# liyi14/mx-DeepIM

Measured on NVIDIA H100. Metric: 480x640 4-iter pose refinements/sec, higher is better.
Workload: dtype fp16

## Files before the change

### mx-deepim_b200/csrc/conv_igemm.cuh

```cuda
#pragma once
#include <cuda.h>
#include <cuda_fp16.h>
#include "common.cuh"
#include "wgmma.cuh"

namespace dim {

struct ConvKParams {
  CUtensorMap a_map[4];
  CUtensorMap a_lo_map[4];
  CUtensorMap b_map;
  CUtensorMap b_lo_map;
  CUtensorMap out_map[2];
  const __nv_bfloat16 *in_hi, *in_lo;
  int in_cols;
  int KH, KW, stride, cchunks;
  int BW, BH, n_col_tiles;
  int Hq, Ho, Wo, Bn;
  int out_Hp, out_Wp, out_py, out_px, Cout;
  int kblocks;
  float slope;
  const float *bias;
  __nv_bfloat16 *out_hi, *out_lo;
  int in_off_r, in_off_c;
// ... 139 lines not shown

constexpr int kConv1Slack = 2048;


__device__ __forceinline__ int frag_row(int t) { return ((t >> 5) << 4) + ((t & 31) >> 2); }

__device__ __forceinline__ uint32_t pack2_bf16_lo(float v0, float v1, uint32_t hi) {
  return pack2_bf16(v0 - __uint_as_float(hi << 16), v1 - __uint_as_float(hi & 0xFFFF0000u));
}

template <bool SPLIT3, bool F16>
__device__ __forceinline__ void epi_pack(float v0, float v1, float b0, float b1, float slope, uint32_t &hi, uint32_t &lo) {
  v0 += b0;
  v1 += b1;
  v0 = v0 > 0.f ? v0 : v0 * slope;
  v1 = v1 > 0.f ? v1 : v1 * slope;
  if (F16) {
    hi = pack2_f16(v0, v1);
  } else {
    hi = pack2_bf16(v0, v1);
    if (SPLIT3) lo = pack2_bf16_lo(v0, v1, hi);
  }
}

template <bool SPLIT3, bool F16>
__device__ __forceinline__ void store_pair(float v0, float v1, float2 b, float slope, __nv_bfloat16 *out_hi, __nv_bfloat16 *out_lo,
                                           long long off) {
  uint32_t h, l = 0;
  epi_pack<SPLIT3, F16>(v0, v1, b.x, b.y, slope, h, l);
  *reinterpret_cast<uint32_t *>(out_hi + off) = h;
  if (SPLIT3) *reinterpret_cast<uint32_t *>(out_lo + off) = l;
}

template <bool SPLIT3>
__device__ __forceinline__ void store_pair_generic(float v0, float v1, const ConvKParams &p, int n, bool valid, long long off,
                                                   long long add_off, long long mask_off) {
  if (!valid || n >= p.Cout) return;
  if (p.bias) {
    v0 += __ldg(p.bias + n);
    v1 += __ldg(p.bias + n + 1);
  }
  if (p.addend.p) {
    const __nv_bfloat162 a = *reinterpret_cast<const __nv_bfloat162 *>(p.addend.p + add_off);
    if (SPLIT3) {
      const __nv_bfloat162 al = *reinterpret_cast<const __nv_bfloat162 *>(p.addend.lo + add_off);
      v0 += __low2float(a) + __low2float(al);
      v1 += __high2float(a) + __high2float(al);
    } else {
      v0 += __low2float(a);
      v1 += __high2float(a);
    }
  }
  if (p.mask.p) {
    if (n < p.mask_climit) {
      const __nv_bfloat162 m = *reinterpret_cast<const __nv_bfloat162 *>(p.mask.p + mask_off);
      if (!(__low2float(m) > 0.f)) v0 *= p.slope;
      if (!(__high2float(m) > 0.f)) v1 *= p.slope;
    }
  } else {
    v0 = v0 > 0.f ? v0 : v0 * p.slope;
    v1 = v1 > 0.f ? v1 : v1 * p.slope;
  }
  if (SPLIT3) {
    const uint32_t h = pack2_bf16(v0, v1);
    *reinterpret_cast<uint32_t *>(p.out_hi + off) = h;
    *reinterpret_cast<uint32_t *>(p.out_lo + off) = pack2_bf16_lo(v0, v1, h);
  } else {
    *reinterpret_cast<__nv_bfloat162 *>(p.out_hi + off) = __floats2bfloat162_rn(v0, v1);
  }
}

template <int BLOCK_N, int STAGES, bool SPLIT3, int EPI>
struct ConvSmem2 {
  static constexpr int A_BYTES = 128 * 64 * 2;
  static constexpr int B_BYTES = BLOCK_N * 64 * 2;
  static constexpr int NPREC = SPLIT3 ? 2 : 1;
  static constexpr int STAGE_BYTES = (A_BYTES + B_BYTES) * NPREC;
  static constexpr int RING_BYTES = STAGES * STAGE_BYTES;
  static constexpr int LIMIT = 227 * 1024, FIXED = 1024  + 256 ;
  static constexpr bool TMA_EPI = EPI == 0 && !SPLIT3;
  static constexpr int STG_GROUPS =
      !TMA_EPI ? 0 : (RING_BYTES + 2 * BLOCK_N * 128 + FIXED <= LIMIT ? BLOCK_N / 64 : BLOCK_N / 128);
  static constexpr int STG_ROUNDS = TMA_EPI ? BLOCK_N / 64 / STG_GROUPS : 0;
  static constexpr int STG_BYTES = STG_GROUPS * 8192;
  static constexpr int TOTAL = RING_BYTES + 2 * STG_BYTES + FIXED;
  static_assert(TOTAL <= LIMIT, "conv_igemm shared memory");
};

template <int BLOCK_N, int STAGES, bool SPLIT3, bool F16, int EPI = 0>
__global__ void __launch_bounds__(384, 1) conv_igemm_persistent_kernel(const __grid_constant__ ConvKParams p,
                                                                       const int total_tiles, const int n_tiles) {
  using S = ConvSmem2<BLOCK_N, STAGES, SPLIT3, EPI>;
  constexpr uint32_t SBO = 1024u;

  extern __shared__ uint8_t smem_raw[];
  uint8_t *smem = reinterpret_cast<uint8_t *>((reinterpret_cast<uintptr_t>(smem_raw) + 1023) & ~(uintptr_t)1023);
  uint8_t *stg = smem + S::RING_BYTES;
  uint64_t *full_bar = reinterpret_cast<uint64_t *>(stg + 2 * S::STG_BYTES);
  uint64_t *empty_bar = full_bar + STAGES;

  const int wgi = threadIdx.x >> 7, warp = threadIdx.x >> 5;

  if (threadIdx.x == 0) {
    for (int s = 0; s < STAGES; ++s) {
      ptx::mbar_init(&full_bar[s], 1);
      ptx::mbar_init(&empty_bar[s], 2);
    }
    ptx::fence_barrier_init();
    ptx::prefetch_tmap(&p.b_map);
    ptx::prefetch_tmap(&p.a_map[0]);
    if (S::TMA_EPI) ptx::prefetch_tmap(&p.out_map[0]);
  }
  __syncthreads();

  if (wgi == 0) {
    ptx::regs_producer();
    if (warp == 0) {
      const uint32_t tx = (uint32_t)(p.BW * p.BH * 64 * 2 + BLOCK_N * 64 * 2) * S::NPREC;
      int s = 0;
      uint32_t ph = 0;
      for (int tile = blockIdx.x; tile < total_tiles; tile += gridDim.x) {
        const int nt = tile % n_tiles, mt = tile / n_tiles;
        const int col_tile = mt % p.n_col_tiles, row_tile = mt / p.n_col_tiles;
        const int g0 = row_tile * p.BH, ow0 = col_tile * p.BW, n0 = nt * BLOCK_N;
        for (int kb = 0; kb < p.kblocks; ++kb) {
          ptx::mbar_wait(&empty_bar[s], ph ^ 1u);
// ... 3 lines not shown
          if (p.stride == 2) {
            view = ((kh & 1) << 1) | (kw & 1);
            dr = kh >> 1;
            dc = kw >> 1;
          }
          uint8_t *st = smem + s * S::STAGE_BYTES;
          if (EPI) { dr += p.in_off_r; dc += p.in_off_c; }
          if (ptx::elect_one()) {
            ptx::mbar_expect_tx_raw(&full_bar[s], tx);
            for (int pr = 0; pr < S::NPREC; ++pr) {
              uint8_t *sa = st + pr * (S::A_BYTES + S::B_BYTES);
              const CUtensorMap *am = pr ? &p.a_lo_map[view] : &p.a_map[view];
              ptx::tma_load_3d_raw(sa, am, &full_bar[s], cc * 64, ow0 + dc, g0 + dr);
              if (EPI == 0) ptx::tma_load_3d_raw(sa + S::A_BYTES / 2, am, &full_bar[s], cc * 64, ow0 + dc, g0 + dr + (p.BH >> 1));
              ptx::tma_load_2d_raw(sa + S::A_BYTES, pr ? &p.b_lo_map : &p.b_map, &full_bar[s], kb * 64, n0);
            }
          }
          __syncwarp();
          if (++s == STAGES) { s = 0; ph ^= 1u; }
        }
      }
    }
  } else {
    ptx::regs_consumer();
    const int t = threadIdx.x & 127;
    const int half = wgi - 1;
    const int q2 = (t & 3) * 2;
    const bool arriver = t == 0;
    const uint32_t base = ptx::smem_u32(smem);
    uint8_t *my_stg = stg + half * S::STG_BYTES;
    const int lane = t & 31;
    const uint32_t st_addr = ptx::smem_u32(my_stg) + (uint32_t)((16 * (t >> 5) + 8 * ((lane >> 3) & 1) + (lane & 7)) * 128);
    const uint32_t st_sw = (uint32_t)(((lane >> 4) & 1) ^ (lane & 7));
    float acc[BLOCK_N / 2];
    int s = 0;
    uint32_t ph = 0;
    for (int tile = blockIdx.x; tile < total_tiles; tile += gridDim.x) {
      int prev = -1;
      for (int kb = 0; kb < p.kblocks; ++kb) {
        ptx::mbar_wait(&full_bar[s], ph);
        const uint32_t a_hi = base + s * S::STAGE_BYTES + half * 8192;
        const uint32_t b_hi = base + s * S::STAGE_BYTES + S::A_BYTES;
        const uint64_t da0 = ptx::gmma_desc(a_hi, 16, SBO, ptx::kSW128), db0 = ptx::gmma_desc(b_hi, 16, SBO, ptx::kSW128);
        const uint64_t dal0 = da0 + ((S::A_BYTES + S::B_BYTES) >> 4), dbl0 = db0 + ((S::A_BYTES + S::B_BYTES) >> 4);
        wg::fence_acc(acc);
        wg::fence();
#pragma unroll
        for (int k = 0; k < 4; ++k) {
          const uint64_t da = da0 + (uint64_t)(2 * k), db = db0 + (uint64_t)(2 * k);
          wg::mma<BLOCK_N, F16, 0, 0>(acc, da, db, (kb > 0 || k > 0) ? 1u : 0u);
          if (SPLIT3) {
            wg::mma<BLOCK_N, false, 0, 0>(acc, dal0 + (uint64_t)(2 * k), db, 1u);
            wg::mma<BLOCK_N, false, 0, 0>(acc, da, dbl0 + (uint64_t)(2 * k), 1u);
          }
        }
        wg::commit();
        wg::wait<1>();
        wg::fence_acc(acc);
        if (prev >= 0 && arriver) ptx::mbar_arrive(&empty_bar[prev]);
        prev = s;
        if (++s == STAGES) { s = 0; ph ^= 1u; }
      }
      wg::wait<0>();
      wg::fence_acc(acc);
      if (prev >= 0 && arriver) ptx::mbar_arrive(&empty_bar[prev]);

      const int nt = tile % n_tiles, mt = tile / n_tiles;
      const int col_tile = mt % p.n_col_tiles, row_tile = mt / p.n_col_tiles;
      const int n0 = nt * BLOCK_N;
      if constexpr (S::TMA_EPI) {
        const int gs = row_tile * p.BH + half * (p.BH >> 1), ow0 = col_tile * p.BW;
        const int n_img = gs / p.Hq, oh = gs - n_img * p.Hq;
        const bool store0 = n_img < p.Bn && oh < p.Ho, store1 = n_img + 1 < p.Bn && oh + (p.BH >> 1) > p.Hq;
#pragma unroll
        for (int rd = 0; rd < S::STG_ROUNDS; ++rd) {
          if (arriver) ptx::bulk_wait_read0();
          ptx::named_bar_sync(1 + half, 128);
#pragma unroll
          for (int i = 0; i < S::STG_GROUPS * 4; ++i) {
            const int j = rd * S::STG_GROUPS * 8 + 2 * i;
            const float *bj = p.bias + n0 + 8 * j + q2;
            const float b0 = __ldg(bj), b1 = __ldg(bj + 1), b2 = __ldg(bj + 8), b3 = __ldg(bj + 9);
            uint32_t h[4], unused;
            epi_pack<false, F16>(acc[4 * j + 0], acc[4 * j + 1], b0, b1, p.slope, h[0], unused);
            epi_pack<false, F16>(acc[4 * j + 2], acc[4 * j + 3], b0, b1, p.slope, h[1], unused);
            epi_pack<false, F16>(acc[4 * j + 4], acc[4 * j + 5], b2, b3, p.slope, h[2], unused);
            epi_pack<false, F16>(acc[4 * j + 6], acc[4 * j + 7], b2, b3, p.slope, h[3], unused);
            ptx::stmatrix_x4(st_addr + (uint32_t)((i >> 2) * 8192) + (((uint32_t)(2 * (i & 3)) ^ st_sw) << 4), h);
          }
          ptx::fence_proxy_async();
          ptx::named_bar_sync(1 + half, 128);
          if (arriver && store0) {
            for (int q = 0; q < S::STG_GROUPS; ++q)
              ptx::tma_store_4d(&p.out_map[0], my_stg + q * 8192, n0 + (rd * S::STG_GROUPS + q) * 64, ow0, oh, n_img);
            ptx::bulk_commit();
          }
        }
        if (store1) {
#pragma unroll
          for (int rr = 0; rr < 2; ++rr) {
            const int lr = frag_row(t) + rr * 8, bh = lr / p.BW;
            const int oh1 = oh + bh - p.Hq, ow = ow0 + lr - bh * p.BW;
            if (lr < p.BW * (p.BH >> 1) && oh1 >= 0 && oh1 < p.Ho) {
// ... 102 lines not shown
    if (warp == 0 && n_rows > 0) {
      if (ptx::elect_one()) {
        ptx::mbar_expect_tx_raw(res_bar, (uint32_t)S::RES_BYTES);
        for (int kb = 0; kb < 16; ++kb) {
          ptx::tma_load_2d_raw(res + kb * S::TAP_BYTES, &p.b_map, res_bar, kb * 32, 0);
          if (SPLIT3) ptx::tma_load_2d_raw(res + (16 + kb) * S::TAP_BYTES, &p.b_lo_map, res_bar, kb * 32, 0);
        }
      }
      __syncwarp();
      const size_t plane = (size_t)p.in_cols * 16;
      const uint8_t *src_hi = reinterpret_cast<const uint8_t *>(p.in_hi) + (size_t)ow0 * 16;
      const uint8_t *src_lo = reinterpret_cast<const uint8_t *>(p.in_lo) + (size_t)ow0 * 16;
      for (int s = 0; s < n_strips; ++s) {
        const int slot = s % STAGES;
        ptx::mbar_wait(&empty_bar[slot], (((uint32_t)(s / STAGES)) & 1u) ^ 1u);
        uint8_t *st = ring + slot * S::STAGE_BYTES;
        if (g_lo + s >= rows_total) {
          if (ptx::elect_one()) ptx::mbar_arrive(&full_bar[slot]);
        } else if (ptx::elect_one()) {
          ptx::mbar_expect_tx_raw(&full_bar[slot], (uint32_t)(4 * S::PLANE_BYTES * S::NPREC));
          const size_t row = (size_t)(g_lo + s) * 4 * plane;
#pragma unroll
          for (int c = 0; c < 4; ++c) {
            ptx::bulk_load_raw(st + c * S::PLANE_BYTES, src_hi + row + c * plane, S::PLANE_BYTES, &full_bar[slot]);
            if (SPLIT3)
              ptx::bulk_load_raw(st + S::STRIP_BYTES + c * S::PLANE_BYTES, src_lo + row + c * plane, S::PLANE_BYTES, &full_bar[slot]);
          }
        }
        __syncwarp();
      }
    }
  } else if (n_rows > 0) {
    ptx::regs_consumer();
    const int set = wgi - 1, t = threadIdx.x & 127, lane = t & 31;
    const bool leader = t == 0;
    const int co = frag_row(t);
    const float b0 = __ldg(p.bias + co), b1 = __ldg(p.bias + co + 8);
    const uint32_t ring_a = ptx::smem_u32(ring);
    const uint64_t dring = ptx::gmma_desc(ring_a, S::PLANE_BYTES, 128, ptx::kNoSwizzle);
    const uint64_t dring3 = ptx::gmma_desc(ring_a, 2u * S::PLANE_BYTES, 128, ptx::kNoSwizzle) + 3u;
    const uint64_t lo_step = (uint64_t)(S::STRIP_BYTES >> 4);
    const uint64_t slot_step = (uint64_t)(S::STAGE_BYTES >> 4);
    const uint64_t kstep = (uint64_t)(2 * S::PLANE_BYTES >> 4);
    const uint64_t dres = ptx::gmma_desc(ptx::smem_u32(res), 16, 512, ptx::kSW64);
    const uint64_t dres_lo = dres + (uint64_t)((16 * S::TAP_BYTES) >> 4);
    uint8_t *my_stg = stg + set * S::NPREC * S::STG_BYTES;
    const int st_px = ((lane >> 4) << 3) + (lane & 7), st_chunk = 2 * (t >> 5) + ((lane >> 3) & 1);
    const uint32_t st_addr = ptx::smem_u32(my_stg) + (uint32_t)(st_px * 128 + ((st_chunk ^ (lane & 7)) << 4));
    ptx::mbar_wait(res_bar, 0);
    if (set == 1 && leader) ptx::mbar_arrive(&empty_bar[0]);
    for (int row = set; row < n_rows; row += 2) {
      float acc[N / 2];
#pragma unroll
      for (int dh = 0; dh < 4; ++dh) {
        const int s = row + dh;
        ptx::mbar_wait(&full_bar[s % STAGES], ((uint32_t)(s / STAGES)) & 1u);
      }
      wg::fence_acc(acc);
      wg::fence();
#pragma unroll
      for (int dh = 0; dh < 4; ++dh) {
        const uint64_t so = (uint64_t)((row + dh) % STAGES) * slot_step;
#pragma unroll
        for (int k = 0; k < 2; ++k) {
#pragma unroll
          for (int dw = 0; dw < 4; ++dw) {
            if ((dh == 3 || dw == 3) && k == 1) continue;
            const uint64_t db = (dw == 3 ? dring3 : dring + (uint64_t)dw + (uint64_t)k * kstep) + so;
            const uint64_t wo = (uint64_t)((dh * 4 + dw) * (S::TAP_BYTES >> 4) + 2 * k);
            wg::mma<N, F16, 0, 0>(acc, dres + wo, db, (dh | dw | k) ? 1u : 0u);
            if (SPLIT3) {
              wg::mma<N, false, 0, 0>(acc, dres + wo, db + lo_step, 1u);
              wg::mma<N, false, 0, 0>(acc, dres_lo + wo, db, 1u);
            }
          }
        }
      }
      wg::commit();
      wg::wait<0>();
      wg::fence_acc(acc);
      if (leader) {
        ptx::mbar_arrive(&empty_bar[row % STAGES]);
        ptx::mbar_arrive(&empty_bar[(row + 1) % STAGES]);
      }
      const int g = g_lo + row;
      const int n_img = g / p.Hq, oh = g - n_img * p.Hq;
      if (n_img < p.Bn && oh < p.Ho) {
        if (leader) ptx::bulk_wait_read0();
        ptx::named_bar_sync(1 + set, 128);
#pragma unroll
        for (int i = 0; i < N / 16; ++i) {
          uint32_t h[4], l[4] = {0, 0, 0, 0};
          epi_pack<SPLIT3, F16>(acc[8 * i + 0], acc[8 * i + 1], b0, b0, p.slope, h[0], l[0]);
          epi_pack<SPLIT3, F16>(acc[8 * i + 2], acc[8 * i + 3], b1, b1, p.slope, h[1], l[1]);
          epi_pack<SPLIT3, F16>(acc[8 * i + 4], acc[8 * i + 5], b0, b0, p.slope, h[2], l[2]);
          epi_pack<SPLIT3, F16>(acc[8 * i + 6], acc[8 * i + 7], b1, b1, p.slope, h[3], l[3]);
          ptx::stmatrix_x4_trans(st_addr + (uint32_t)(i * 16 * 128), h);
          if (SPLIT3) ptx::stmatrix_x4_trans(st_addr + (uint32_t)(S::STG_BYTES + i * 16 * 128), l);
        }
        ptx::fence_proxy_async();
        ptx::named_bar_sync(1 + set, 128);
        if (leader) {
#pragma unroll
          for (int q = 0; q < N / kConv1StoreN; ++q) {
            ptx::tma_store_4d(&p.out_map[0], my_stg + q * kConv1StoreN * 128, 0, ow0 + q * kConv1StoreN, oh, n_img);
            if (SPLIT3)
              ptx::tma_store_4d(&p.out_map[1], my_stg + S::STG_BYTES + q * kConv1StoreN * 128, 0, ow0 + q * kConv1StoreN, oh, n_img);
          }
          ptx::bulk_commit();
        }
      }
    }
    if (leader) ptx::bulk_wait0();
  }
}

template <int STAGES, bool SPLIT3, bool F16, int NB>
__global__ void __launch_bounds__(384, 1) conv1_rgbd_kernel(const __grid_constant__ ConvKParams p, const int rows_total,
                                                            const int rows_per_chunk, const int chunks_per_col,
                                                            const int strip_bytes ) {
  constexpr int NPREC = SPLIT3 ? 2 : 1;
  constexpr int TAP_BYTES = NB * 128, RES_BYTES = 16 * TAP_BYTES * NPREC;
  extern __shared__ uint8_t smem_raw[];
  uint8_t *smem = reinterpret_cast<uint8_t *>((reinterpret_cast<uintptr_t>(smem_raw) + 1023) & ~(uintptr_t)1023);
  uint8_t *res = smem;
  uint8_t *ring = smem + RES_BYTES;
  const int stage_bytes = strip_bytes * NPREC;
  uint64_t *full_bar = reinterpret_cast<uint64_t *>(ring + STAGES * stage_bytes + kConv1Slack);
  uint64_t *empty_bar = full_bar + STAGES;
  uint64_t *res_bar = empty_bar + STAGES;

  const int wgi = threadIdx.x >> 7, warp = threadIdx.x >> 5;
// ... 127 lines not shown
```

### mx-deepim_b200/csrc/net.cu

```cuda
#include <cuda_fp16.h>
#include <string.h>

#include <memory>
#include <mutex>

#include "launch.cuh"
#include "net_state.cuh"

namespace dim {

static void build_geometry(NetState *ns, int H, int W) {
  int h = H, w = W;
  for (int i = 0; i < 10; ++i) {
    const LayerSpec &s = kLayers[i];
    LayerGeom &g = ns->g[i];
    g.Cin = s.Cin; g.Cout = s.Cout; g.k = s.k; g.stride = s.stride; g.pad = s.pad;
    g.Hin = h; g.Win = w;
    g.Ho = (h + 2 * s.pad - s.k) / s.stride + 1;
    g.Wo = (w + 2 * s.pad - s.k) / s.stride + 1;
    if (g.Ho < 1) g.Ho = 1;
    if (g.Wo < 1) g.Wo = 1;
    int Hp = h + 2 * s.pad, Wp = w + 2 * s.pad;
    if (s.stride == 2) { Hp += Hp & 1; Wp += Wp & 1; }
    g.py = g.px = s.pad;
// ... 2 lines not shown
      g.rows = Hp / 2; g.cols = Wp / 2; g.Cbuf = 64;
      g.KH = g.KW = 4; g.stride_eff = 1; g.Ceff = 64; g.Hq = g.rows;
      g.BLOCK_K = 64; g.BLOCK_N = 64;
    } else if (i == 0) {
      g.rows = Hp / 2; g.cols = Wp / 2; g.Cbuf = 32;
      g.KH = g.KW = 4; g.stride_eff = 1; g.Ceff = 32; g.Hq = g.rows;
      g.BLOCK_K = 32; g.BLOCK_N = 64;
    } else {
      g.rows = Hp; g.cols = Wp; g.Cbuf = s.Cin;
      g.KH = g.KW = s.k; g.stride_eff = s.stride; g.Ceff = s.Cin;
      g.Hq = (s.stride == 2) ? Hp / 2 : Hp;
      g.BLOCK_K = 64; g.BLOCK_N = s.Cout >= 256 ? 256 : 128;
    }
    int best_bw = 0, best_score = -1;
    for (int pass = 0; pass < 2 && best_bw == 0; ++pass)
      for (int d = 1; d <= g.Wo && d <= 128; ++d) {
        if (g.Wo % d) continue;
        if (pass == 0 && d < 8) continue;
        const int score = d * (128 / d) * 1000 + d;
        if (score > best_score) { best_score = score; best_bw = d; }
      }
    if (best_bw == 0) best_bw = 1;
    g.BW = best_bw; g.BH = 128 / best_bw;
    g.n_col_tiles = g.Wo > 0 ? g.Wo / g.BW : 0;
    if (i == 0) {
      const int nt = cdiv(g.Wo, 128);
      g.BW = cdiv(g.Wo, nt); g.BH = 1; g.n_col_tiles = nt;
    }
    g.kblocks = g.KH * g.KW * (g.Ceff / g.BLOCK_K);
    h = g.Ho; w = g.Wo;
  }
}

typedef CUresult (*EncodeTiledFn)(CUtensorMap *, CUtensorMapDataType, cuuint32_t, void *, const cuuint64_t *,
                                  const cuuint64_t *, const cuuint32_t *, const cuuint32_t *, CUtensorMapInterleave,
                                  CUtensorMapSwizzle, CUtensorMapL2promotion, CUtensorMapFloatOOBfill);
static EncodeTiledFn get_encode() {
  static EncodeTiledFn fn = nullptr;
  if (!fn) {
    void *p = nullptr;
    cudaDriverEntryPointQueryResult q;
    if (cudaGetDriverEntryPoint("cuTensorMapEncodeTiled", &p, cudaEnableDefault, &q) == cudaSuccess &&
        q == cudaDriverEntryPointSuccess)
      fn = reinterpret_cast<EncodeTiledFn>(p);
  }
  return fn;
}

int encode_map(CUtensorMap *m, void *base, int rank, const uint64_t *dims, const uint64_t *strides_bytes,
                      const uint32_t *box, int block_k ) {
  EncodeTiledFn fn = get_encode();
  DIM_REQUIRE(fn != nullptr, "cuTensorMapEncodeTiled entry point not available (driver too old?)");
  cuuint64_t gd[5]; cuuint64_t gs[5]; cuuint32_t bx[5]; cuuint32_t es[5];
  for (int i = 0; i < rank; ++i) { gd[i] = dims[i]; bx[i] = box[i]; es[i] = 1; }
  for (int i = 0; i < rank - 1; ++i) gs[i] = strides_bytes[i];
  CUresult r = fn(m, CU_TENSOR_MAP_DATA_TYPE_BFLOAT16, (cuuint32_t)rank, base, gd, gs, bx, es,
                  CU_TENSOR_MAP_INTERLEAVE_NONE,
                  block_k == 64 ? CU_TENSOR_MAP_SWIZZLE_128B
                                : (block_k == 32 ? CU_TENSOR_MAP_SWIZZLE_64B : CU_TENSOR_MAP_SWIZZLE_NONE),
                  CU_TENSOR_MAP_L2_PROMOTION_L2_256B, CU_TENSOR_MAP_FLOAT_OOB_FILL_NONE);
  if (r != CUDA_SUCCESS) {
    set_error("cuTensorMapEncodeTiled failed with CUresult %d (rank %d dims %llu %llu %llu box %u %u %u)", (int)r, rank,
              (unsigned long long)dims[0], (unsigned long long)dims[1], (unsigned long long)(rank > 2 ? dims[2] : 0),
              box[0], box[1], rank > 2 ? box[2] : 0);
    return 3;
  }
  return 0;
}

static int build_maps(NetState *ns, int B, bool f16, TensorMaps &tm) {
  for (int i = 0; i < 10; ++i) {
    const LayerGeom &g = ns->g[i];
    ConvKParams &kp = tm.kp[i];
    memset(&kp, 0, sizeof(kp));
    for (int lo = 0; lo < 2; ++lo) {
      __nv_bfloat16 *base = lo ? ns->act_lo[i] : ns->act_hi[i];
      CUtensorMap *maps = lo ? kp.a_lo_map : kp.a_map;
      const uint32_t box[3] = {(uint32_t)g.BLOCK_K, (uint32_t)g.BW, (uint32_t)(g.BH / 2)};
      if (i == 0 && ns->input_depth) {
        const uint64_t dims[4] = {8, (uint64_t)g.cols, 8, (uint64_t)B * g.rows};
        const uint64_t str[3] = {16, (uint64_t)g.cols * 16, (uint64_t)g.cols * 128};
        const uint32_t box4[4] = {8, (uint32_t)(g.BW + 3), 8, 1};
        if (int rc = encode_map(&maps[0], base, 4, dims, str, box4, 0)) return rc;
        maps[1] = maps[2] = maps[3] = maps[0];
      } else if (i == 0) {
      } else if (g.stride_eff == 1) {
        const uint64_t dims[3] = {(uint64_t)g.Cbuf, (uint64_t)g.cols, (uint64_t)B * g.rows};
        const uint64_t str[2] = {(uint64_t)g.Cbuf * 2, (uint64_t)g.cols * g.Cbuf * 2};
        if (int rc = encode_map(&maps[0], base, 3, dims, str, box, g.BLOCK_K)) return rc;
        maps[1] = maps[2] = maps[3] = maps[0];
      } else {
        for (int ph = 0; ph < 2; ++ph)
          for (int pw = 0; pw < 2; ++pw) {
            const uint64_t dims[3] = {(uint64_t)g.Cbuf, (uint64_t)g.cols / 2, (uint64_t)B * g.rows / 2};
            const uint64_t str[2] = {(uint64_t)2 * g.Cbuf * 2, (uint64_t)2 * g.cols * g.Cbuf * 2};
            __nv_bfloat16 *vb = base + ((size_t)ph * g.cols + pw) * g.Cbuf;
            if (int rc = encode_map(&maps[(ph << 1) | pw], vb, 3, dims, str, box, g.BLOCK_K)) return rc;
          }
      }
    }
    {
      const uint64_t Ktot = (uint64_t)g.KH * g.KW * g.Ceff;
      const uint64_t dims[2] = {Ktot, (uint64_t)g.Cout};
      const uint64_t str[1] = {Ktot * 2};
      const uint32_t box[2] = {(uint32_t)g.BLOCK_K, (uint32_t)(i == 0 && ns->input_depth ? 16 : g.BLOCK_N)};
      __nv_bfloat16 *wop = f16 ? ns->w_f16[i] : ns->w_hi[i];
      if (int rc = encode_map(&kp.b_map, wop, 2, dims, str, box, g.BLOCK_K)) return rc;
      if (int rc = encode_map(&kp.b_lo_map, ns->w_lo[i], 2, dims, str, box, g.BLOCK_K)) return rc;
    }
    kp.KH = g.KH; kp.KW = g.KW; kp.stride = g.stride_eff; kp.cchunks = g.Ceff / g.BLOCK_K;
    kp.BW = g.BW; kp.BH = g.BH; kp.n_col_tiles = g.n_col_tiles;
    kp.Hq = g.Hq; kp.Ho = g.Ho; kp.Wo = g.Wo; kp.Bn = B;
    if (i < 9) {
      const LayerGeom &nx = ns->g[i + 1];
      kp.out_Hp = nx.rows; kp.out_Wp = nx.cols; kp.out_py = nx.py; kp.out_px = nx.px;
    } else {
      kp.out_Hp = g.Ho; kp.out_Wp = g.Wo; kp.out_py = 0; kp.out_px = 0;
    }
    kp.Cout = g.Cout;
    kp.kblocks = g.kblocks;
    kp.slope = 0.1f;
    kp.bias = ns->bias[i];
    kp.out_hi = ns->act_hi[i + 1];
    kp.out_lo = ns->act_lo[i + 1];
    if (i == 0 && !ns->input_depth) {
      kp.in_hi = ns->act_hi[0];
      kp.in_lo = ns->act_lo[0];
      kp.in_cols = g.cols;
    }
    if (i > 0 || !ns->input_depth) {
      DIM_REQUIRE(i == 0 || (g.BH % 2 == 0 && g.BH / 2 <= g.Hq && g.BW * (g.BH / 2) <= 64),
                  "conv_igemm: a consumer warpgroup's box must be whole output rows within two images");
      const uint64_t cb = (uint64_t)g.Cout * 2;
      const uint64_t dims[4] = {(uint64_t)g.Cout, (uint64_t)g.Wo, (uint64_t)g.Ho, (uint64_t)B};
      const uint64_t str[3] = {cb, (uint64_t)kp.out_Wp * cb, (uint64_t)kp.out_Hp * kp.out_Wp * cb};
      const uint32_t box[4] = {64, (uint32_t)(i == 0 ? kConv1StoreN : g.BW), (uint32_t)(i == 0 ? 1 : g.BH / 2), 1};
      const size_t interior = ((size_t)kp.out_py * kp.out_Wp + kp.out_px) * g.Cout;
      for (int lo = 0; lo < (i == 0 ? 2 : 1); ++lo)
        if (int rc = encode_map(&kp.out_map[lo], (lo ? ns->act_lo[i + 1] : ns->act_hi[i + 1]) + interior, 4, dims, str, box, 64))
          return rc;
    }
  }
  return 0;
}

template <bool F16>
__device__ __forceinline__ void mma_bf16_16816(float *c, const uint32_t *a, uint32_t b0, uint32_t b1) {
  if (F16)
    asm volatile(
        "mma.sync.aligned.m16n8k16.row.col.f32.f16.f16.f32 {%0,%1,%2,%3}, {%4,%5,%6,%7}, {%8,%9}, {%0,%1,%2,%3};"
        : "+f"(c[0]), "+f"(c[1]), "+f"(c[2]), "+f"(c[3])
        : "r"(a[0]), "r"(a[1]), "r"(a[2]), "r"(a[3]), "r"(b0), "r"(b1));
  else
    asm volatile(
        "mma.sync.aligned.m16n8k16.row.col.f32.bf16.bf16.f32 {%0,%1,%2,%3}, {%4,%5,%6,%7}, {%8,%9}, {%0,%1,%2,%3};"
        : "+f"(c[0]), "+f"(c[1]), "+f"(c[2]), "+f"(c[3])
        : "r"(a[0]), "r"(a[1]), "r"(a[2]), "r"(a[3]), "r"(b0), "r"(b1));
}

template <bool S3, bool F16 = false>
__global__ void __launch_bounds__(256) fc6_mma_kernel(const __nv_bfloat16 *__restrict__ act_hi,
                                                      const __nv_bfloat16 *__restrict__ act_lo,
                                                      const __nv_bfloat16 *__restrict__ w_hi,
                                                      const __nv_bfloat16 *__restrict__ w_lo, int B, int max_batch,
                                                      float *__restrict__ partial) {
  constexpr int PITCH = FC6_KC * 2 + 64;
  __shared__ __align__(16) uint8_t a_hi_s[16 * PITCH];
  __shared__ __align__(16) uint8_t a_lo_s[S3 ? 16 * PITCH : 16];
  const int s = blockIdx.x, k0 = s * FC6_KC;
// ... 273 lines not shown
  n[11] = 256 * 256;
  for (int i = 0; i < 12; ++i) off[i + 1] = off[i] + n[i];
  float *stage_p = nullptr;
  DIM_CHECK(cudaMalloc(&stage_p, off[12] * sizeof(float)));
  std::unique_ptr<float, cudaError_t (*)(void *)> stage(stage_p, cudaFree);
  auto put = [](float *dst, const float *src, size_t count) {
    return cudaMemcpy(dst, src, count * sizeof(float), cudaMemcpyHostToDevice);
  };
  const float *w[12];
  for (int i = 0; i < 12; ++i) {
    w[i] = stage.get() + off[i];
    if (i != 10) DIM_CHECK(put(stage.get() + off[i], W[i], n[i]));
  }
  {
    std::vector<float> p((size_t)256 * FC6_K);
    for (int o = 0; o < 256; ++o)
      for (int c = 0; c < 1024; ++c)
        for (int hw = 0; hw < 80; ++hw) p[(size_t)o * FC6_K + (size_t)hw * 1024 + c] = W[10][(size_t)o * FC6_K + (size_t)c * 80 + hw];
    DIM_CHECK(put(stage.get() + off[10], p.data(), n[10]));
  }
  for (int i = 0; i < 10; ++i) DIM_CHECK(put(ns->bias[i], Bv[i], ns->g[i].Cout));
  DIM_CHECK(put(ns->fc6_b, Bv[10], 256));
  DIM_CHECK(put(ns->fc7_b, Bv[11], 256));
  DIM_CHECK(put(ns->rot_w, W[12], 4 * 256));
  DIM_CHECK(put(ns->rot_b, Bv[12], 4));
  DIM_CHECK(put(ns->trans_w, W[13], 3 * 256));
  DIM_CHECK(put(ns->trans_b, Bv[13], 3));
  if (int rc = net_pack_weights(ctx, w, 0, true, true)) return rc;
  DIM_CHECK(cudaStreamSynchronize(0));
  ns->loaded = true;
  return 0;
}

template <int BN, int ST, bool S3, bool F16>
static int launch_conv(const ConvKParams &kp, int total_tiles, int n_tiles, int cap, cudaStream_t st) {
  using S = ConvSmem2<BN, ST, S3, 0>;
  static bool attr_set = false;
  if (!attr_set) {
    DIM_CHECK(cudaFuncSetAttribute(conv_igemm_persistent_kernel<BN, ST, S3, F16>, cudaFuncAttributeMaxDynamicSharedMemorySize,
                                   S::TOTAL));
    attr_set = true;
  }
  const int grid = total_tiles < cap ? total_tiles : cap;
  conv_igemm_persistent_kernel<BN, ST, S3, F16><<<grid, 384, S::TOTAL, st>>>(kp, total_tiles, n_tiles);
  DIM_LAUNCH_CHECK();
  return 0;
}

template <int N, int ST, bool S3, bool F16>
static int launch_conv1(const ConvKParams &kp, int grid, int rows_total, int rpc, int chunks, cudaStream_t st) {
  using S = Conv1Smem<N, ST, S3>;
  static bool set = false;
  if (!set) {
    DIM_CHECK(cudaFuncSetAttribute(conv1_kernel<N, ST, S3, F16>, cudaFuncAttributeMaxDynamicSharedMemorySize, S::TOTAL));
    set = true;
  }
  conv1_kernel<N, ST, S3, F16><<<grid, 384, S::TOTAL, st>>>(kp, rows_total, rpc, chunks);
  DIM_LAUNCH_CHECK();
  return 0;
}

template <int ST, bool S3, bool F16, int NB>
static int launch_conv1_rgbd(const ConvKParams &kp, int grid, int rows_total, int rpc, int chunks, int strip_bytes,
                             cudaStream_t st) {
  const int smem_bytes = 16 * NB * 128 * (S3 ? 2 : 1) + ST * (S3 ? 2 : 1) * strip_bytes + kConv1Slack + 1024 + 256;
  DIM_REQUIRE(smem_bytes <= 227 * 1024, "conv1 (RGB-D): image too wide for the rolling-strip ring");
  static int set = 0;
  if (set < smem_bytes) {
    DIM_CHECK(cudaFuncSetAttribute(conv1_rgbd_kernel<ST, S3, F16, NB>, cudaFuncAttributeMaxDynamicSharedMemorySize,
                                   smem_bytes));
    set = smem_bytes;
  }
  conv1_rgbd_kernel<ST, S3, F16, NB><<<grid, 384, smem_bytes, st>>>(kp, rows_total, rpc, chunks, strip_bytes);
  DIM_LAUNCH_CHECK();
  return 0;
}

// ... 15 lines not shown
  }
  ns->act_hi[0] = enable ? ns->act0_rgbd_hi : ns->act0_rgb_hi;
  ns->act_lo[0] = enable ? ns->act0_rgbd_lo : ns->act0_rgb_lo;
  return 0;
}

bool net_input_depth(dim_ctx *ctx) { return ctx->net && ctx->net->input_depth; }

int net_set_input_mask(dim_ctx *ctx, bool enable) {
  NetState *ns = ctx->net;
  DIM_REQUIRE(ns != nullptr, "net not created");
  if (ns->input_mask == enable) return 0;
  DIM_REQUIRE(!ns->loaded, "dim_ctx_set_input_mask: call it before dim_net_load (this context's weights are loaded)");
  ns->input_mask = enable;
  return 0;
}

bool net_input_mask(dim_ctx *ctx) { return !ctx->net || ctx->net->input_mask; }

void net_input_geometry(dim_ctx *ctx, int *rows, int *cols, int *pad, __nv_bfloat16 **hi, __nv_bfloat16 **lo) {
  NetState *ns = ctx->net;
  *rows = ns->g[0].rows; *cols = ns->g[0].cols; *pad = ns->g[0].py;
  *hi = ns->act_hi[0]; *lo = ns->act_lo[0];
}

int net_forward(dim_ctx *ctx, int B, int precision, const float *zoom_factor, float *rot_out, float *trans_out,
                float *se3_out, cudaStream_t st, cudaEvent_t after_conv) {
  NetState *ns = ctx->net;
  DIM_REQUIRE(ns && ns->loaded, "dim_net_load has not been called");
  DIM_REQUIRE(B >= 1 && B <= ctx->max_batch, "batch exceeds max_batch");
  DIM_REQUIRE(precision == DIM_PREC_BF16 || precision == DIM_PREC_BF16X3 || precision == DIM_PREC_FP16,
              "unknown precision (DIM_PREC_BF16 / DIM_PREC_BF16X3 / DIM_PREC_FP16)");
  const bool s3 = precision == DIM_PREC_BF16X3, f16 = precision == DIM_PREC_FP16;
  const int key = B + (f16 ? kF16MapKey : 0);
  auto it = ns->maps.find(key);
  if (it == ns->maps.end()) {
    TensorMaps tm;
    if (int rc = build_maps(ns, B, f16, tm)) return rc;
    it = ns->maps.emplace(key, tm).first;
  }
  const TensorMaps &tm = it->second;
  if (ns->repack_done) DIM_CHECK(cudaStreamWaitEvent(st, ns->repack_done, 0));
  if (s3 && ns->lo_stale)
    if (int rc = train_refresh_lo(ctx, st)) return rc;
  if (f16 && ns->f16_stale)
    if (int rc = net_refresh_f16(ctx, st)) return rc;
  if (ns->layer_events) DIM_CHECK(cudaEventRecord(ns->layer_events[0], st));
  for (int i = 0; i < 10; ++i) {
    const LayerGeom &g = ns->g[i];
    const ConvKParams &kp = tm.kp[i];
    const int n_tiles = g.Cout / g.BLOCK_N;
    const int total_tiles = cdiv(B * g.Hq, g.BH) * g.n_col_tiles * n_tiles;
    const int sms = ctx->num_sms;
    int rc;
    if (i == 0 && ns->input_depth) {
      const int nsplit = s3 ? 4 : 1;
      const int rows_total = B * g.Hq;
      int chunks = sms / (g.n_col_tiles * nsplit);
      if (chunks > cdiv(rows_total, 16)) chunks = cdiv(rows_total, 16);
      if (chunks < 1) chunks = 1;
      const int rpc = cdiv(rows_total, chunks);
      chunks = cdiv(rows_total, rpc);
      const int strip_bytes = cdiv((g.BW + 3) * 128, 128) * 128;
      const int grid = g.n_col_tiles * chunks * nsplit;
      rc = s3 ? launch_conv1_rgbd<5, true, false, 16>(kp, grid, rows_total, rpc, chunks, strip_bytes, st)
              : (f16 ? launch_conv1_rgbd<6, false, true, 64>(kp, grid, rows_total, rpc, chunks, strip_bytes, st)
                     : launch_conv1_rgbd<6, false, false, 64>(kp, grid, rows_total, rpc, chunks, strip_bytes, st));
    } else if (i == 0) {
      DIM_REQUIRE(g.Wo == 320 && g.cols >= g.Wo + 3 && g.Hq == g.rows && g.Hq == g.Ho + 3,
                  "conv1_kernel is built for a 480x640 input (320 output columns)");
      const int n_col = g.Wo / (s3 ? 80 : 160);
      const int rows_total = B * g.Hq;
      int chunks = sms / n_col;
      if (chunks > cdiv(rows_total, 16)) chunks = cdiv(rows_total, 16);
      if (chunks < 1) chunks = 1;
      const int rpc = cdiv(rows_total, chunks);
      chunks = cdiv(rows_total, rpc);
      const int grid = n_col * chunks;
      rc = s3 ? launch_conv1<80, 5, true, false>(kp, grid, rows_total, rpc, chunks, st)
              : (f16 ? launch_conv1<160, 8, false, true>(kp, grid, rows_total, rpc, chunks, st)
                     : launch_conv1<160, 8, false, false>(kp, grid, rows_total, rpc, chunks, st));
    } else if (g.BLOCK_N == 128) {
      rc = s3 ? launch_conv<128, 3, true, false>(kp, total_tiles, n_tiles, sms, st)
              : (f16 ? launch_conv<128, 6, false, true>(kp, total_tiles, n_tiles, sms, st)
                     : launch_conv<128, 6, false, false>(kp, total_tiles, n_tiles, sms, st));
    } else {
      rc = s3 ? launch_conv<256, 2, true, false>(kp, total_tiles, n_tiles, sms, st)
              : (f16 ? launch_conv<256, 4, false, true>(kp, total_tiles, n_tiles, sms, st)
                     : launch_conv<256, 4, false, false>(kp, total_tiles, n_tiles, sms, st));
    }
    if (rc) return rc;
    if (ns->layer_events && i < 9) DIM_CHECK(cudaEventRecord(ns->layer_events[i + 1], st));
  }
  if (ns->layer_events) DIM_CHECK(cudaEventRecord(ns->layer_events[10], st));
  if (after_conv) DIM_CHECK(cudaEventRecord(after_conv, st));
  if (s3)
    fc6_mma_kernel<true><<<FC6_SPLITS, 256, 0, st>>>(ns->act_hi[10], ns->act_lo[10], ns->fc6_w_hi, ns->fc6_w_lo, B,
                                                     ctx->max_batch, ns->fc6_partial);
  else if (f16)
    fc6_mma_kernel<false, true><<<FC6_SPLITS, 256, 0, st>>>(ns->act_hi[10], nullptr, ns->fc6_w_f16, nullptr, B,
                                                            ctx->max_batch, ns->fc6_partial);
  else
    fc6_mma_kernel<false><<<FC6_SPLITS, 256, 0, st>>>(ns->act_hi[10], nullptr, ns->fc6_w_hi, nullptr, B,
                                                      ctx->max_batch, ns->fc6_partial);
  DIM_LAUNCH_CHECK();
  head_kernel<<<B, 1024, 0, st>>>(ns->fc6_partial, ctx->max_batch, ns->fc6_b, ns->fc7_wT, ns->fc7_b, ns->rot_w,
                                 ns->rot_b, ns->trans_w, ns->trans_b, zoom_factor, rot_out, trans_out, se3_out, ns->save_h6,
                                 ns->save_h7);
  DIM_LAUNCH_CHECK();
  return 0;
}

bool net_graph_safe(dim_ctx *ctx) {
  NetState *ns = ctx->net;
  return ns && ns->loaded && !ns->layer_events && !ns->train_aliased;
}

int net_layer_profile(dim_ctx *ctx, int enable, float *ms10) {
// ... 41 lines not shown
```

### mx-deepim_b200/csrc/net_state.cuh

```cuda
#pragma once
#include <map>

#include "conv_igemm.cuh"

namespace dim {

struct LayerSpec {
  const char *name;
  int Cout, Cin, k, stride, pad;
};
static const LayerSpec kLayers[10] = {
    {"flow_conv1", 64, 8, 7, 2, 3},  {"conv2", 128, 64, 5, 2, 2},   {"conv3", 256, 128, 5, 2, 2},
    {"conv3_1", 256, 256, 3, 1, 1},  {"conv4", 512, 256, 3, 2, 1},  {"conv4_1", 512, 512, 3, 1, 1},
    {"conv5", 512, 512, 3, 2, 1},    {"conv5_1", 512, 512, 3, 1, 1}, {"conv6", 1024, 512, 3, 2, 1},
    {"conv6_1", 1024, 1024, 3, 1, 1}};

struct LayerGeom {
  int Cin, Cout, k, stride, pad, Hin, Win, Ho, Wo;
  int rows, cols, Cbuf, py, px;
  int KH, KW, stride_eff, Ceff, Hq;
  int BLOCK_N, BLOCK_K, BW, BH, n_col_tiles, kblocks;
};

struct TensorMaps {
// ... 14 lines not shown
  LayerGeom g[10];
  __nv_bfloat16 *w_hi[10] = {}, *w_lo[10] = {};
  __nv_bfloat16 *w_f16[10] = {};
  float *bias[10] = {};
  __nv_bfloat16 *act_hi[11] = {}, *act_lo[11] = {};
  size_t act_elems_per_image[11] = {};
  __nv_bfloat16 *fc6_w_hi = nullptr, *fc6_w_lo = nullptr;
  __nv_bfloat16 *fc6_w_f16 = nullptr;
  bool train_aliased = false;
  bool f16_stale = false;
  float *fc6_b = nullptr, *fc7_wT = nullptr, *fc7_b = nullptr, *rot_w = nullptr, *rot_b = nullptr,
        *trans_w = nullptr, *trans_b = nullptr;
  float *fc6_partial = nullptr;
  cudaEvent_t *layer_events = nullptr;
  bool loaded = false, net_ok = false;
  bool input_depth = false;
  __nv_bfloat16 *act0_rgb_hi = nullptr, *act0_rgb_lo = nullptr, *act0_rgbd_hi = nullptr, *act0_rgbd_lo = nullptr;
  bool input_mask = true;
  float *save_h6 = nullptr, *save_h7 = nullptr;
  cudaEvent_t repack_done = nullptr;
  bool lo_stale = false;
  std::map<int, TensorMaps> maps;
  int max_batch = 0;
};

static constexpr int FC6_K = 1024 * 8 * 10;
static constexpr int FC6_KC = 256;
static constexpr int FC6_SPLITS = FC6_K / FC6_KC;


int encode_map(CUtensorMap *m, void *base, int rank, const uint64_t *dims, const uint64_t *strides_bytes,
               const uint32_t *box, int block_k );
static constexpr int kF16MapKey = 1 << 20;

}
```

Baseline: 3316.

## Transpose 128-channel conv GEMM so weights are M and 256 pixels are N

For 128-output-channel layers in fp16/bf16 forward mode, the implicit-GEMM kernel swaps operands: each consumer warpgroup takes 64 output channels as the MMA M dimension and a 256-pixel tile as N. The accumulator is written through stmatrix-transposed staging and TMA-stored one output row at a time. Doubling the pixel tile is meant to reuse each weight tile across more pixels and give larger wgmma N, at the cost of fewer pipeline stages (6 to 4), more accumulator registers, and per-row TMA stores issued by one thread. Tensor-map caching now keys on bf16x3 so the differing tile geometry stays separate.

```diff
diff --git a/mx-deepim_b200/csrc/conv_igemm.cuh b/mx-deepim_b200/csrc/conv_igemm.cuh
--- a/mx-deepim_b200/csrc/conv_igemm.cuh
+++ b/mx-deepim_b200/csrc/conv_igemm.cuh
@@ -195,6 +195,22 @@
   if (SPLIT3) *reinterpret_cast<uint32_t *>(out_lo + off) = l;
 }
 
+__device__ __forceinline__ uint32_t stage_trans_lane(int t) {
+  const int lane = t & 31;
+  const int px = ((lane >> 4) << 3) + (lane & 7), chunk = 2 * (t >> 5) + ((lane >> 3) & 1);
+  return (uint32_t)(px * 128 + ((chunk ^ (lane & 7)) << 4));
+}
+template <bool SPLIT3, bool F16>
+__device__ __forceinline__ void stage_trans16(const float *a, float b0, float b1, float slope, uint32_t addr, uint32_t lo_off) {
+  uint32_t h[4], l[4] = {0, 0, 0, 0};
+  epi_pack<SPLIT3, F16>(a[0], a[1], b0, b0, slope, h[0], l[0]);
+  epi_pack<SPLIT3, F16>(a[2], a[3], b1, b1, slope, h[1], l[1]);
+  epi_pack<SPLIT3, F16>(a[4], a[5], b0, b0, slope, h[2], l[2]);
+  epi_pack<SPLIT3, F16>(a[6], a[7], b1, b1, slope, h[3], l[3]);
+  ptx::stmatrix_x4_trans(addr, h);
+  if (SPLIT3) ptx::stmatrix_x4_trans(addr + lo_off, l);
+}
+
 template <bool SPLIT3>
 __device__ __forceinline__ void store_pair_generic(float v0, float v1, const ConvKParams &p, int n, bool valid, long long off,
                                                    long long add_off, long long mask_off) {
@@ -233,28 +249,32 @@
   }
 }
 
-template <int BLOCK_N, int STAGES, bool SPLIT3, int EPI>
+template <int BLOCK_N, int STAGES, bool SPLIT3, int EPI, bool TRANS = false>
 struct ConvSmem2 {
-  static constexpr int A_BYTES = 128 * 64 * 2;
+  static constexpr int TILE_PX = TRANS ? 256 : 128;
+  static constexpr int A_BYTES = TILE_PX * 64 * 2;
   static constexpr int B_BYTES = BLOCK_N * 64 * 2;
   static constexpr int NPREC = SPLIT3 ? 2 : 1;
   static constexpr int STAGE_BYTES = (A_BYTES + B_BYTES) * NPREC;
   static constexpr int RING_BYTES = STAGES * STAGE_BYTES;
   static constexpr int LIMIT = 227 * 1024, FIXED = 1024  + 256 ;
   static constexpr bool TMA_EPI = EPI == 0 && !SPLIT3;
+  static constexpr int OUT_BLOCKS = (TRANS ? TILE_PX : BLOCK_N) / 64;
   static constexpr int STG_GROUPS =
-      !TMA_EPI ? 0 : (RING_BYTES + 2 * BLOCK_N * 128 + FIXED <= LIMIT ? BLOCK_N / 64 : BLOCK_N / 128);
-  static constexpr int STG_ROUNDS = TMA_EPI ? BLOCK_N / 64 / STG_GROUPS : 0;
+      !TMA_EPI ? 0 : (RING_BYTES + 2 * OUT_BLOCKS * 8192 + FIXED <= LIMIT ? OUT_BLOCKS : OUT_BLOCKS / 2);
+  static constexpr int STG_ROUNDS = TMA_EPI ? OUT_BLOCKS / STG_GROUPS : 0;
   static constexpr int STG_BYTES = STG_GROUPS * 8192;
   static constexpr int TOTAL = RING_BYTES + 2 * STG_BYTES + FIXED;
   static_assert(TOTAL <= LIMIT, "conv_igemm shared memory");
+  static_assert(!TRANS || (BLOCK_N == 128 && TMA_EPI), "transposed tiles: 128 output channels, fp16 / bf16 forward");
 };
 
-template <int BLOCK_N, int STAGES, bool SPLIT3, bool F16, int EPI = 0>
+template <int BLOCK_N, int STAGES, bool SPLIT3, bool F16, int EPI = 0, bool TRANS = false>
 __global__ void __launch_bounds__(384, 1) conv_igemm_persistent_kernel(const __grid_constant__ ConvKParams p,
                                                                        const int total_tiles, const int n_tiles) {
-  using S = ConvSmem2<BLOCK_N, STAGES, SPLIT3, EPI>;
+  using S = ConvSmem2<BLOCK_N, STAGES, SPLIT3, EPI, TRANS>;
   constexpr uint32_t SBO = 1024u;
+  constexpr int MMA_N = TRANS ? S::TILE_PX : BLOCK_N;
 
   extern __shared__ uint8_t smem_raw[];
   uint8_t *smem = reinterpret_cast<uint8_t *>((reinterpret_cast<uintptr_t>(smem_raw) + 1023) & ~(uintptr_t)1023);
@@ -324,15 +344,17 @@
     const int lane = t & 31;
     const uint32_t st_addr = ptx::smem_u32(my_stg) + (uint32_t)((16 * (t >> 5) + 8 * ((lane >> 3) & 1) + (lane & 7)) * 128);
     const uint32_t st_sw = (uint32_t)(((lane >> 4) & 1) ^ (lane & 7));
-    float acc[BLOCK_N / 2];
+    const uint32_t st_trans = ptx::smem_u32(my_stg) + stage_trans_lane(t);
+    float acc[MMA_N / 2];
     int s = 0;
     uint32_t ph = 0;
     for (int tile = blockIdx.x; tile < total_tiles; tile += gridDim.x) {
       int prev = -1;
       for (int kb = 0; kb < p.kblocks; ++kb) {
         ptx::mbar_wait(&full_bar[s], ph);
-        const uint32_t a_hi = base + s * S::STAGE_BYTES + half * 8192;
-        const uint32_t b_hi = base + s * S::STAGE_BYTES + S::A_BYTES;
+        const uint32_t act = base + s * S::STAGE_BYTES, wts = act + S::A_BYTES;
+        const uint32_t a_hi = TRANS ? wts + half * 8192 : act + half * 8192;
+        const uint32_t b_hi = TRANS ? act : wts;
         const uint64_t da0 = ptx::gmma_desc(a_hi, 16, SBO, ptx::kSW128), db0 = ptx::gmma_desc(b_hi, 16, SBO, ptx::kSW128);
         const uint64_t dal0 = da0 + ((S::A_BYTES + S::B_BYTES) >> 4), dbl0 = db0 + ((S::A_BYTES + S::B_BYTES) >> 4);
         wg::fence_acc(acc);
@@ -340,10 +362,10 @@
 #pragma unroll
         for (int k = 0; k < 4; ++k) {
           const uint64_t da = da0 + (uint64_t)(2 * k), db = db0 + (uint64_t)(2 * k);
-          wg::mma<BLOCK_N, F16, 0, 0>(acc, da, db, (kb > 0 || k > 0) ? 1u : 0u);
+          wg::mma<MMA_N, F16, 0, 0>(acc, da, db, (kb > 0 || k > 0) ? 1u : 0u);
           if (SPLIT3) {
-            wg::mma<BLOCK_N, false, 0, 0>(acc, dal0 + (uint64_t)(2 * k), db, 1u);
-            wg::mma<BLOCK_N, false, 0, 0>(acc, da, dbl0 + (uint64_t)(2 * k), 1u);
+            wg::mma<MMA_N, false, 0, 0>(acc, dal0 + (uint64_t)(2 * k), db, 1u);
+            wg::mma<MMA_N, false, 0, 0>(acc, da, dbl0 + (uint64_t)(2 * k), 1u);
           }
         }
         wg::commit();
@@ -360,7 +382,29 @@
       const int nt = tile % n_tiles, mt = tile / n_tiles;
       const int col_tile = mt % p.n_col_tiles, row_tile = mt / p.n_col_tiles;
       const int n0 = nt * BLOCK_N;
-      if constexpr (S::TMA_EPI) {
+      if constexpr (TRANS) {
+        constexpr int RPX = S::STG_GROUPS * 64;
+        const int c0 = n0 + 64 * half + frag_row(t), rows = RPX / p.BW, ow0 = col_tile * p.BW;
+        const float b0 = __ldg(p.bias + c0), b1 = __ldg(p.bias + c0 + 8);
+#pragma unroll
+        for (int rd = 0; rd < S::STG_ROUNDS; ++rd) {
+          if (arriver) ptx::bulk_wait_read0();
+          ptx::named_bar_sync(1 + half, 128);
+#pragma unroll
+          for (int i = 0; i < RPX / 16; ++i)
+            stage_trans16<false, F16>(acc + 8 * (rd * (RPX / 16) + i), b0, b1, p.slope, st_trans + (uint32_t)(i * 16 * 128), 0);
+          ptx::fence_proxy_async();
+          ptx::named_bar_sync(1 + half, 128);
+          if (arriver) {
+            for (int r = 0; r < rows; ++r) {
+              const int g = row_tile * p.BH + rd * rows + r, n_img = g / p.Hq, oh = g - n_img * p.Hq;
+              if (n_img < p.Bn && oh < p.Ho)
+                ptx::tma_store_4d(&p.out_map[0], my_stg + r * p.BW * 128, n0 + 64 * half, ow0, oh, n_img);
+            }
+            ptx::bulk_commit();
+          }
+        }
+      } else if constexpr (S::TMA_EPI) {
         const int gs = row_tile * p.BH + half * (p.BH >> 1), ow0 = col_tile * p.BW;
         const int n_img = gs / p.Hq, oh = gs - n_img * p.Hq;
         const bool store0 = n_img < p.Bn && oh < p.Ho, store1 = n_img + 1 < p.Bn && oh + (p.BH >> 1) > p.Hq;
@@ -529,7 +573,7 @@
     }
   } else if (n_rows > 0) {
     ptx::regs_consumer();
-    const int set = wgi - 1, t = threadIdx.x & 127, lane = t & 31;
+    const int set = wgi - 1, t = threadIdx.x & 127;
     const bool leader = t == 0;
     const int co = frag_row(t);
     const float b0 = __ldg(p.bias + co), b1 = __ldg(p.bias + co + 8);
@@ -542,8 +586,7 @@
     const uint64_t dres = ptx::gmma_desc(ptx::smem_u32(res), 16, 512, ptx::kSW64);
     const uint64_t dres_lo = dres + (uint64_t)((16 * S::TAP_BYTES) >> 4);
     uint8_t *my_stg = stg + set * S::NPREC * S::STG_BYTES;
-    const int st_px = ((lane >> 4) << 3) + (lane & 7), st_chunk = 2 * (t >> 5) + ((lane >> 3) & 1);
-    const uint32_t st_addr = ptx::smem_u32(my_stg) + (uint32_t)(st_px * 128 + ((st_chunk ^ (lane & 7)) << 4));
+    const uint32_t st_addr = ptx::smem_u32(my_stg) + stage_trans_lane(t);
     ptx::mbar_wait(res_bar, 0);
     if (set == 1 && leader) ptx::mbar_arrive(&empty_bar[0]);
     for (int row = set; row < n_rows; row += 2) {
@@ -586,15 +629,8 @@
         if (leader) ptx::bulk_wait_read0();
         ptx::named_bar_sync(1 + set, 128);
 #pragma unroll
-        for (int i = 0; i < N / 16; ++i) {
-          uint32_t h[4], l[4] = {0, 0, 0, 0};
-          epi_pack<SPLIT3, F16>(acc[8 * i + 0], acc[8 * i + 1], b0, b0, p.slope, h[0], l[0]);
-          epi_pack<SPLIT3, F16>(acc[8 * i + 2], acc[8 * i + 3], b1, b1, p.slope, h[1], l[1]);
-          epi_pack<SPLIT3, F16>(acc[8 * i + 4], acc[8 * i + 5], b0, b0, p.slope, h[2], l[2]);
-          epi_pack<SPLIT3, F16>(acc[8 * i + 6], acc[8 * i + 7], b1, b1, p.slope, h[3], l[3]);
-          ptx::stmatrix_x4_trans(st_addr + (uint32_t)(i * 16 * 128), h);
-          if (SPLIT3) ptx::stmatrix_x4_trans(st_addr + (uint32_t)(S::STG_BYTES + i * 16 * 128), l);
-        }
+        for (int i = 0; i < N / 16; ++i)
+          stage_trans16<SPLIT3, F16>(acc + 8 * i, b0, b1, p.slope, st_addr + (uint32_t)(i * 16 * 128), S::STG_BYTES);
         ptx::fence_proxy_async();
         ptx::named_bar_sync(1 + set, 128);
         if (leader) {
diff --git a/mx-deepim_b200/csrc/net.cu b/mx-deepim_b200/csrc/net.cu
--- a/mx-deepim_b200/csrc/net.cu
+++ b/mx-deepim_b200/csrc/net.cu
@@ -58,6 +58,8 @@
   }
 }
 
+static bool fwd_transposed(const LayerGeom &g, bool s3) { return g.BLOCK_N == 128 && !s3; }
+
 typedef CUresult (*EncodeTiledFn)(CUtensorMap *, CUtensorMapDataType, cuuint32_t, void *, const cuuint64_t *,
                                   const cuuint64_t *, const cuuint32_t *, const cuuint32_t *, CUtensorMapInterleave,
                                   CUtensorMapSwizzle, CUtensorMapL2promotion, CUtensorMapFloatOOBfill);
@@ -94,15 +96,17 @@
   return 0;
 }
 
-static int build_maps(NetState *ns, int B, bool f16, TensorMaps &tm) {
+static int build_maps(NetState *ns, int B, bool f16, bool s3, TensorMaps &tm) {
   for (int i = 0; i < 10; ++i) {
     const LayerGeom &g = ns->g[i];
     ConvKParams &kp = tm.kp[i];
     memset(&kp, 0, sizeof(kp));
+    const bool trans = i > 0 && fwd_transposed(g, s3);
+    const int BH = trans ? 2 * g.BH : g.BH;
     for (int lo = 0; lo < 2; ++lo) {
       __nv_bfloat16 *base = lo ? ns->act_lo[i] : ns->act_hi[i];
       CUtensorMap *maps = lo ? kp.a_lo_map : kp.a_map;
-      const uint32_t box[3] = {(uint32_t)g.BLOCK_K, (uint32_t)g.BW, (uint32_t)(g.BH / 2)};
+      const uint32_t box[3] = {(uint32_t)g.BLOCK_K, (uint32_t)g.BW, (uint32_t)(BH / 2)};
       if (i == 0 && ns->input_depth) {
         const uint64_t dims[4] = {8, (uint64_t)g.cols, 8, (uint64_t)B * g.rows};
         const uint64_t str[3] = {16, (uint64_t)g.cols * 16, (uint64_t)g.cols * 128};
@@ -135,7 +139,7 @@
       if (int rc = encode_map(&kp.b_lo_map, ns->w_lo[i], 2, dims, str, box, g.BLOCK_K)) return rc;
     }
     kp.KH = g.KH; kp.KW = g.KW; kp.stride = g.stride_eff; kp.cchunks = g.Ceff / g.BLOCK_K;
-    kp.BW = g.BW; kp.BH = g.BH; kp.n_col_tiles = g.n_col_tiles;
+    kp.BW = g.BW; kp.BH = BH; kp.n_col_tiles = g.n_col_tiles;
     kp.Hq = g.Hq; kp.Ho = g.Ho; kp.Wo = g.Wo; kp.Bn = B;
     if (i < 9) {
       const LayerGeom &nx = ns->g[i + 1];
@@ -155,12 +159,14 @@
       kp.in_cols = g.cols;
     }
     if (i > 0 || !ns->input_depth) {
-      DIM_REQUIRE(i == 0 || (g.BH % 2 == 0 && g.BH / 2 <= g.Hq && g.BW * (g.BH / 2) <= 64),
+      DIM_REQUIRE(i == 0 || trans || (g.BH % 2 == 0 && g.BH / 2 <= g.Hq && g.BW * (g.BH / 2) <= 64),
                   "conv_igemm: a consumer warpgroup's box must be whole output rows within two images");
+      DIM_REQUIRE(!trans || (g.BW * g.BH == 128 && g.BW % 8 == 0),
+                  "conv_igemm (transposed): the 256-pixel tile must be whole rows of a multiple of 8 pixels dividing 128");
       const uint64_t cb = (uint64_t)g.Cout * 2;
       const uint64_t dims[4] = {(uint64_t)g.Cout, (uint64_t)g.Wo, (uint64_t)g.Ho, (uint64_t)B};
       const uint64_t str[3] = {cb, (uint64_t)kp.out_Wp * cb, (uint64_t)kp.out_Hp * kp.out_Wp * cb};
-      const uint32_t box[4] = {64, (uint32_t)(i == 0 ? kConv1StoreN : g.BW), (uint32_t)(i == 0 ? 1 : g.BH / 2), 1};
+      const uint32_t box[4] = {64, (uint32_t)(i == 0 ? kConv1StoreN : g.BW), (uint32_t)(i == 0 || trans ? 1 : g.BH / 2), 1};
       const size_t interior = ((size_t)kp.out_py * kp.out_Wp + kp.out_px) * g.Cout;
       for (int lo = 0; lo < (i == 0 ? 2 : 1); ++lo)
         if (int rc = encode_map(&kp.out_map[lo], (lo ? ns->act_lo[i + 1] : ns->act_hi[i + 1]) + interior, 4, dims, str, box, 64))
@@ -500,17 +506,17 @@
   return 0;
 }
 
-template <int BN, int ST, bool S3, bool F16>
+template <int BN, int ST, bool S3, bool F16, bool TRANS = false>
 static int launch_conv(const ConvKParams &kp, int total_tiles, int n_tiles, int cap, cudaStream_t st) {
-  using S = ConvSmem2<BN, ST, S3, 0>;
+  using S = ConvSmem2<BN, ST, S3, 0, TRANS>;
   static bool attr_set = false;
   if (!attr_set) {
-    DIM_CHECK(cudaFuncSetAttribute(conv_igemm_persistent_kernel<BN, ST, S3, F16>, cudaFuncAttributeMaxDynamicSharedMemorySize,
-                                   S::TOTAL));
+    DIM_CHECK(cudaFuncSetAttribute(conv_igemm_persistent_kernel<BN, ST, S3, F16, 0, TRANS>,
+                                   cudaFuncAttributeMaxDynamicSharedMemorySize, S::TOTAL));
     attr_set = true;
   }
   const int grid = total_tiles < cap ? total_tiles : cap;
-  conv_igemm_persistent_kernel<BN, ST, S3, F16><<<grid, 384, S::TOTAL, st>>>(kp, total_tiles, n_tiles);
+  conv_igemm_persistent_kernel<BN, ST, S3, F16, 0, TRANS><<<grid, 384, S::TOTAL, st>>>(kp, total_tiles, n_tiles);
   DIM_LAUNCH_CHECK();
   return 0;
 }
@@ -592,11 +598,11 @@
   DIM_REQUIRE(precision == DIM_PREC_BF16 || precision == DIM_PREC_BF16X3 || precision == DIM_PREC_FP16,
               "unknown precision (DIM_PREC_BF16 / DIM_PREC_BF16X3 / DIM_PREC_FP16)");
   const bool s3 = precision == DIM_PREC_BF16X3, f16 = precision == DIM_PREC_FP16;
-  const int key = B + (f16 ? kF16MapKey : 0);
+  const int key = B + (f16 ? kF16MapKey : 0) + (s3 ? kBF16X3MapKey : 0);
   auto it = ns->maps.find(key);
   if (it == ns->maps.end()) {
     TensorMaps tm;
-    if (int rc = build_maps(ns, B, f16, tm)) return rc;
+    if (int rc = build_maps(ns, B, f16, s3, tm)) return rc;
     it = ns->maps.emplace(key, tm).first;
   }
   const TensorMaps &tm = it->second;
@@ -610,7 +616,7 @@
     const LayerGeom &g = ns->g[i];
     const ConvKParams &kp = tm.kp[i];
     const int n_tiles = g.Cout / g.BLOCK_N;
-    const int total_tiles = cdiv(B * g.Hq, g.BH) * g.n_col_tiles * n_tiles;
+    const int total_tiles = cdiv(B * g.Hq, kp.BH) * g.n_col_tiles * n_tiles;
     const int sms = ctx->num_sms;
     int rc;
     if (i == 0 && ns->input_depth) {
@@ -642,8 +648,8 @@
                      : launch_conv1<160, 8, false, false>(kp, grid, rows_total, rpc, chunks, st));
     } else if (g.BLOCK_N == 128) {
       rc = s3 ? launch_conv<128, 3, true, false>(kp, total_tiles, n_tiles, sms, st)
-              : (f16 ? launch_conv<128, 6, false, true>(kp, total_tiles, n_tiles, sms, st)
-                     : launch_conv<128, 6, false, false>(kp, total_tiles, n_tiles, sms, st));
+              : (f16 ? launch_conv<128, 4, false, true, true>(kp, total_tiles, n_tiles, sms, st)
+                     : launch_conv<128, 4, false, false, true>(kp, total_tiles, n_tiles, sms, st));
     } else {
       rc = s3 ? launch_conv<256, 2, true, false>(kp, total_tiles, n_tiles, sms, st)
               : (f16 ? launch_conv<256, 4, false, true>(kp, total_tiles, n_tiles, sms, st)
diff --git a/mx-deepim_b200/csrc/net_state.cuh b/mx-deepim_b200/csrc/net_state.cuh
--- a/mx-deepim_b200/csrc/net_state.cuh
+++ b/mx-deepim_b200/csrc/net_state.cuh
@@ -70,5 +70,6 @@
 int encode_map(CUtensorMap *m, void *base, int rank, const uint64_t *dims, const uint64_t *strides_bytes,
                const uint32_t *box, int block_k );
 static constexpr int kF16MapKey = 1 << 20;
+static constexpr int kBF16X3MapKey = 1 << 21;
 
 }
```

Measured after the change: 3399 (median of 6 runs). 2.5% higher.
